# martius-lab/iCEM

Measured on AMD Instinct MI355X. Metric: traj-steps/sec (N x h), iCEM inner planning loop, higher is better.
Workload: dtype f32 storage; model step 2xfp16 planes (3 products), f32 accumulate

## Files before the change

### icem_amd/build.py

```python
import hashlib
import json
import os
import subprocess
import sys
from concurrent.futures import ThreadPoolExecutor

HERE = os.path.dirname(os.path.abspath(__file__))
CSRC = os.path.join(HERE, "csrc")
UNITS = ["generic_kernels.hip", "plan.hip", "abi.hip", "exchange.hip", "k_sample.hip", "k_rollout.hip", "k_merge.hip",
         "k_iter_small.hip", "icem_rssm.hip", "icem_rssm_split.hip", "k_rollout_wide.hip", "collective.hip", "k_rollout_ahead.hip",
         "k_rollout_wide_split.hip", "k_rollout_hn.hip"]
OUT = os.path.join(HERE, "libicem_hip.so")
OUT_FAULTS = os.path.join(HERE, "libicem_hip_faults.so")
FAULT_UNIT = "exchange.hip"
MARK = b"ICEM_BUILD_HASH="
OBJ = os.path.join(CSRC, "_obj")
FLAGS = ["--offload-arch=gfx950", "-O3", "-std=c++17", "-fPIC", "-Wno-unused-function"]
UNIT_FLAGS = {}
if os.environ.get("ICEM_DEV_SHAPES"):
    FLAGS.append(f"-DICEM_FAST_SHAPES(X)=X({os.environ['ICEM_DEV_SHAPES']})")


def _hipcc() -> str:
    return os.environ.get("HIPCC", "/opt/rocm/bin/hipcc")


def _units():
    return [u for u in UNITS if os.path.exists(os.path.join(CSRC, u))]


def _headers():
    hs = sorted(os.path.join(CSRC, f) for f in os.listdir(CSRC) if f.endswith(".h"))
    return hs + [os.path.join(os.path.dirname(HERE), "include", "icem_hip.h")]


def _digest(paths, extra=""):
    m = hashlib.sha256(extra.encode())
    for p in paths:
        m.update(os.path.basename(p).encode())
        with open(p, "rb") as f:
            m.update(f.read())
    return m.hexdigest()[:16]


def source_hash() -> str:
    return _digest([os.path.join(CSRC, u) for u in _units()] + _headers(), " ".join(FLAGS) + repr(sorted(UNIT_FLAGS.items())))


def embedded_hash(path: str = OUT):
    try:
        with open(path, "rb") as f:
            blob = f.read()
    except OSError:
        return None
    at = blob.find(MARK)
    if at < 0:
        return None
    tag = blob[at + len(MARK):at + len(MARK) + 16]
    return tag.decode() if len(tag) == 16 and all(c in b"0123456789abcdef" for c in tag) else None


def build_info() -> dict:
    info = {"source_hash": source_hash(), "built_from": embedded_hash(), "stale": True}
    info["stale"] = info["built_from"] != info["source_hash"]
    return info


def up_to_date() -> bool:
    return not build_info()["stale"]


def _object(unit, headers_digest, faults=False):
    src = os.path.join(CSRC, unit)
    extra = [f'-DICEM_BUILD_HASH="{source_hash()}"'] if unit == "abi.hip" else []
    if faults:
        extra.append("-DICEM_FAULT_INJECTION")
    cmd = [_hipcc(), *FLAGS, *UNIT_FLAGS.get(unit, []), *extra, "-I", CSRC, "-c", src]
    key = _digest([src], " ".join("csrc" if a == CSRC else a for a in cmd[1:-1]) + headers_digest)
    stem = os.path.splitext(unit)[0] + ("_faults" if faults else "")
    return cmd, os.path.join(OBJ, f"{stem}.{key}.o")


def object_path(unit: str) -> str:
    return _object(unit, _digest(_headers()))[1]


def _compile(unit, headers_digest, verbose, faults=False):
    cmd, obj = _object(unit, headers_digest, faults)
    stem = os.path.splitext(unit)[0] + ("_faults" if faults else "")
    if not os.path.exists(obj):
        for f in os.listdir(OBJ):
            if f.startswith(stem + ".") and f.endswith(".o"):
                os.remove(os.path.join(OBJ, f))
        if verbose:
            print(" ".join(cmd + ["-o", obj]), flush=True)
        subprocess.check_call(cmd + ["-o", obj + ".tmp"])
        os.replace(obj + ".tmp", obj)
    return obj


def build(force: bool = False, verbose: bool = True) -> str:
    if not force and up_to_date() and embedded_hash(OUT_FAULTS) == source_hash():
        return OUT
    os.makedirs(OBJ, exist_ok=True)
    if force:
        for f in os.listdir(OBJ):
            os.remove(os.path.join(OBJ, f))
    hd = _digest(_headers())
    with ThreadPoolExecutor(max_workers=min(8, os.cpu_count() or 1)) as ex:
        fut_faults = ex.submit(_compile, FAULT_UNIT, hd, verbose, True)
        objs = list(ex.map(lambda u: _compile(u, hd, verbose), _units()))
        obj_faults = fut_faults.result()
    objs_f = [obj_faults if os.path.basename(o).startswith(os.path.splitext(FAULT_UNIT)[0] + ".") else o for o in objs]
    for out, oo in ((OUT, objs), (OUT_FAULTS, objs_f)):
        cmd = [_hipcc(), "--offload-arch=gfx950", "-shared", "-fPIC", *oo, "-ldl", "-o", out]
        if verbose:
            print(" ".join(cmd), flush=True)
        subprocess.check_call(cmd)
    if embedded_hash() != source_hash():
        raise RuntimeError("libicem_hip.so does not carry the hash of the sources it was just built from")
    return OUT


if __name__ == "__main__":
    build(force="--force" in sys.argv)
    print(json.dumps(build_info()))
```

### icem_amd/csrc/k_iter_small.hip

```cpp
#include "fused_dev.h"

namespace icem {

namespace {

constexpr bool sr_quad(int d, int rw) { return rw <= 2 && ((4 * 16 * rw * d + 63) / 64) * 64 + 64 <= 1024; }
constexpr int sr_threads(int d, int rw) { return (((sr_quad(d, rw) ? 4 : 1) * 16 * rw * d + 63) / 64) * 64; }

template <int H, int D, int O, int KIND, int ROUNDS, int RW, int KREG, bool REC, int ARITH>
__device__ __forceinline__ void sample_rollout_body(const FastSampleArgs& sa, const FastRolloutArgs& ra, const MergeSingleArgs& am,
                                                    const PackPrev& ap) {
    constexpr bool PM = KREG > 0;
    constexpr bool QS = sr_quad(D, RW);
    constexpr bool T4 = QS && O <= 20 && sr_threads(D, RW) >= 256 * RW && ARITH == 0;
    using T16 = typename TileSel<H, D, O, KIND, ARITH>::type;
    using Tile = typename std::conditional<T4, Tile4<H, D, (O <= 20 ? O : 17), KIND>, T16>::type;
    constexpr int RWV = T4 ? 4 * RW : RW;
    constexpr int HD = H * D;
    constexpr int TPB = 16 * RW;
    constexpr int ROWS = TPB * D;
    constexpr int NT = sr_threads(D, RW);
    constexpr int NTT = NT + (PM ? 64 : 0);
    static_assert(NTT <= 1024 && HD % 2 == 0, "workgroup shape");
    constexpr int VW = HD % 4 == 0 ? 4 : 2;
    using Vec = typename VecOf<VW>::type;
    __shared__ __attribute__((aligned(16))) float ms[2 * HD];
    __shared__ __attribute__((aligned(16))) float tilebuf[T16::SLACK + TPB * HD + T16::TAIL];
    __shared__ unsigned long long wg_keys[2][RW][32];
    __shared__ float obs_stage[32];
    constexpr int WROWS = H / 2 + 1;
    __shared__ __attribute__((aligned(16))) float Wl[QS ? NT / 64 : 1][QS ? WROWS * WQ_STRIDE : 4];
    __shared__ unsigned long long sel[PM ? 64 : 1];
    __shared__ unsigned long long cand[PM ? 64 : 1];
    __shared__ int slot[PM ? 64 : 1];
    float* tile_rows = tilebuf + T16::SLACK;
    const int tid = threadIdx.x;
    const int lane = tid & 63;
    const int wave = tid >> 6;
    const int n_rows = ra.n_rows;
    const bool has_pack = PM && REC && ap.part_k != nullptr;
    if constexpr (PM && REC) {
        if (has_pack && blockIdx.x == 0) {
            MergeSingleArgs pk{};
            pk.n_lists = ap.n_lists;
            pk.n_pool = ap.n_pool;
            pk.n_global = ap.n_global;
            pk.K = ap.K;
            pk.h = H;
            pk.d = D;
            pk.part_k = ap.part_k;
            pk.actions = ap.actions;
            pk.n_keep = ap.n_keep;
            pk.elites_cost_cur = ap.keep_costs;
            pk.keep_base = ap.n_loc;
            __builtin_amdgcn_s_setprio(3);
            if (ra.dbg && tid == 0) ra.dbg[0] = wall_clock64();
            if (tid < 64) {
                if constexpr (NTT <= 512)
                    merge_select<12>(pk, lane, cand, sel);
                else
                    merge_select_stream(pk, lane, cand, sel);
            }
            __syncthreads();
            if (ra.dbg && tid == 0) ra.dbg[1] = wall_clock64();
            pack_records_body<12>(pk, ap.n_loc, ap.shard_lo, ap.records, ap.px, tilebuf, sel, tid, NTT);
            if (ra.dbg && tid == 0) ra.dbg[2] = wall_clock64();
            return;
        }
    }
    const int wg = blockIdx.x - (has_pack ? 1 : 0);
    const int n_wg = ra.list_wgs > 0 ? ra.list_wgs : (int)gridDim.x - (has_pack ? 1 : 0);
    const int base = wg * TPB;
    if (base >= n_rows) return;
    if (ra.dbg && tid == 0 && wg == 0) ra.dbg[8] = wall_clock64();
    const int rowi = QS ? tid >> 2 : tid, q = tid & 3;
    const int nl = rowi / D, jd = rowi - nl * D;
    const bool has_row = rowi < ROWS;
    float* trow = tile_rows + nl * HD + jd;
    const float* mrow = ms + jd;
    Tile tile;
    float obs_reg = 0.f;
    constexpr int WPL = (WROWS * HMAX + 63) / 64;
    float wreg[QS ? WPL : 1];
    const bool pre_drawn = !PM && sa.raw_src != nullptr;
    if constexpr (QS) {
        if (tid < NT && !pre_drawn) {
#pragma unroll
            for (int i = 0; i < WPL; ++i) wreg[i] = sa.W[(i * 64 + lane) < WROWS * HMAX ? i * 64 + lane : 0];
        }
    }
    const int r_mine = base + nl;
    float lo_reg = 0.f, hi_reg = 0.f;
    if ((PM || pre_drawn) && tid < NT) {
        lo_reg = sa.low[jd];
        hi_reg = sa.high[jd];
    }
    constexpr int NVR = !PM ? (TPB * (HD / VW) + NTT - 1) / NTT : 1;
    constexpr int NVB = NVR < 4 ? NVR : 4;
    constexpr int NEL = !PM && QS ? (H - 1 + 3) / 4 : 1;
    typedef float RawV __attribute__((ext_vector_type(VW)));
    RawV rawv[NVB];
    float elv[NEL];
    if (!PM) {
        const int total4 = (n_rows - base < TPB ? n_rows - base : TPB) * (HD / VW);
        RawV* t4 = reinterpret_cast<RawV*>(tile_rows);
        float mreg[(HD + NTT - 1) / NTT], sreg[(HD + NTT - 1) / NTT];
#pragma unroll
        for (int i = 0; i < (HD + NTT - 1) / NTT; ++i) {
            const int e = tid + i * NTT;
            mreg[i] = sa.mean[e < HD ? e : 0];
            sreg[i] = sa.std[e < HD ? e : 0];
        }
        if (pre_drawn) {
            const RawV* g4 = reinterpret_cast<const RawV*>(sa.raw_src + (size_t)base * HD);
#pragma unroll
            for (int i = 0; i < NVB; ++i) {
                const int e = tid + i * NTT;
                rawv[i] = g4[e < total4 ? e : 0];
            }
            if constexpr (QS) {
                if (has_row && tid < NT && r_mine >= sa.n && r_mine < n_rows) {
                    const float* src = sa.elites_src + (size_t)(r_mine - sa.n) * HD + jd;
#pragma unroll
                    for (int i = 0; i < NEL; ++i) elv[i] = src[(q + 4 * i < H - 1 ? q + 4 * i + 1 : 1) * D];
                }
            }
        }
        obs_reg = ra.obs0[(tid < 32 && tid < ra.o) ? tid : 0];
        if (wave < RWV) tile.load(ra, lane);
#pragma unroll
        for (int i = 0; i < (HD + NTT - 1) / NTT; ++i) {
            const int e = tid + i * NTT;
            if (e < HD) {
                ms[e] = mreg[i];
                ms[HD + e] = sreg[i];
            }
        }
        if (pre_drawn) {
#pragma unroll
            for (int i = 0; i < NVB; ++i) {
                const int e = tid + i * NTT;
                if (e < total4) t4[e] = rawv[i];
            }
            if constexpr (NVR > NVB) {
                const RawV* g4 = reinterpret_cast<const RawV*>(sa.raw_src + (size_t)base * HD);
                for (int e0 = tid + NVB * NTT; e0 < total4; e0 += NVB * NTT) {
#pragma unroll
                    for (int i = 0; i < NVB; ++i) rawv[i] = g4[e0 + i * NTT < total4 ? e0 + i * NTT : 0];
#pragma unroll
                    for (int i = 0; i < NVB; ++i)
                        if (e0 + i * NTT < total4) t4[e0 + i * NTT] = rawv[i];
                }
            }
        }
        __syncthreads();
    }
    if (ra.dbg && tid == 0 && wg == 0) ra.dbg[9] = wall_clock64();
    if (pre_drawn) {
        if (has_row && tid < NT) {
            const float lo = lo_reg, hi = hi_reg;
            constexpr int QN = QS ? 4 : 1;
            const int q0 = QS ? q : 0;
            if (r_mine < sa.n) {
                for (int t = q0; t < H; t += QN) {
                    const float v = __builtin_fmaf(trow[t * D], mrow[HD + t * D], mrow[t * D]);
                    trow[t * D] = __builtin_amdgcn_fmed3f(v, lo, hi);
                }
            } else if (r_mine < n_rows) {
                const float* src = sa.elites_src + (size_t)(r_mine - sa.n) * HD + jd;
                if ((H - 1) % QN == q0) {
                    const float v = __builtin_fmaf(trow[(H - 1) * D], mrow[HD + (H - 1) * D], mrow[(H - 1) * D]);
                    trow[(H - 1) * D] = __builtin_amdgcn_fmed3f(v, lo, hi);
                }
                if constexpr (QS) {
#pragma unroll
                    for (int i = 0; i < NEL; ++i)
                        if (q + 4 * i < H - 1) trow[(q + 4 * i) * D] = elv[i];
                } else {
                    for (int t = q0; t < H - 1; t += QN) trow[t * D] = src[(t + 1) * D];
                }
            } else {
                for (int t = q0; t < H; t += QN) trow[t * D] = 0.f;
            }
        }
    } else
    if constexpr (QS) {
        if (tid < NT) {
            float* wl = Wl[wave];
            sample_into_tile_quad<H, D, ROUNDS, PM>(sa, has_row, n_rows, r_mine, jd, q, trow, mrow, wl, [&]() {
#pragma unroll
                for (int i = 0; i < WPL; ++i) {
                    const int e = i * 64 + lane;
                    if (e < WROWS * HMAX) wl[(e / HMAX) * WQ_STRIDE + (e % HMAX)] = wreg[i];
                }
                __builtin_amdgcn_fence(__ATOMIC_RELEASE, "wavefront");
                __builtin_amdgcn_wave_barrier();
                __builtin_amdgcn_fence(__ATOMIC_ACQUIRE, "wavefront");
            });
        }
    } else if (has_row) {
        sample_into_tile<H, D, ROUNDS, PM>(sa, n_rows, r_mine, jd, trow, mrow);
    }
    if constexpr (PM) {
        if (tid >= NT) {
            if constexpr (RW <= 4) __builtin_amdgcn_s_setprio(3);
            if constexpr (REC) {
                if (ra.dbg && lane == 0 && wg == 0) ra.dbg[3] = wall_clock64();
            }
            else if constexpr (RW >= 8)
                merge_select_stream(am, lane, cand, sel);
            else
                merge_select_shallow<3>(am, lane, cand, sel);
        }
    }
    if (PM) {
        obs_reg = ra.obs0[(tid < 32 && tid < ra.o) ? tid : 0];
        if (wave < RWV) tile.load(ra, lane);
    }
    const float* rd0 = nullptr;
    if constexpr (!T4) rd0 = tile.read_ptr(tilebuf + (wave < RW ? wave : 0) * 16 * HD, lane, HD);
    if constexpr (PM) {
        const MergeSingleArgs& m = am;
        if constexpr (REC) {
            merge_select_records_wg(am, tid >= NT, lane, tid, NTT, sel, slot, (ra.dbg && wg == 0) ? ra.dbg + 7 : nullptr);
            if (ra.dbg && tid == 0 && wg == 0) ra.dbg[4] = wall_clock64();
        } else {
            __syncthreads();
        }
        if (ra.dbg && tid == 0 && wg == 0) ra.dbg[5] = wall_clock64();
        if (!REC && ra.dbg && tid == 0 && wg == 0) ra.dbg[15] = wall_clock64();
        const float* rows[KREG > 0 ? KREG : 1];
        merge_rows<KREG, REC>(m, sel, slot, rows);
        for (int e = tid; e < HD; e += NTT) {
            float xs[KREG > 0 ? KREG : 1];
#pragma unroll
            for (int r = 0; r < KREG; ++r) xs[r] = rows[r][e];
            float nm, ns;
            refit_element_regs<float, KREG>(m.K, m.alpha, m.mean[e], m.std[e], xs, nm, ns);
            ms[e] = nm;
            ms[HD + e] = ns;
            if (wg == 0) {
                m.mean_out[e] = nm;
                m.std_out[e] = ns;
#pragma unroll
                for (int r = 0; r < KREG; ++r)
                    if (r < m.K) m.elites_next[(size_t)r * HD + e] = xs[r];
            }
        }
        if (wg == 0 && tid < m.K) m.elites_cost_next[tid] = key_cost(sel[tid]);
        __syncthreads();
        if (ra.dbg && tid == 0 && wg == 0) ra.dbg[6] = wall_clock64();
        if (!REC && ra.dbg && tid == 0 && wg == 0) ra.dbg[7] = wall_clock64();
        if (has_row && r_mine < sa.n) {
            const float lo = lo_reg, hi = hi_reg;
            for (int t = QS ? q : 0; t < H; t += QS ? 4 : 1) {
                const float v = __builtin_fmaf(trow[t * D], mrow[HD + t * D], mrow[t * D]);
                trow[t * D] = __builtin_amdgcn_fmed3f(v, lo, hi);
            }
        }
    }
    if (tid < 32) {
        float ov = obs_reg;
        asm volatile("" : "+v"(ov));
        obs_stage[tid] = tid < ra.o ? ov : 0.f;
    }
    if (ra.dbg && tid == 0 && wg == 0) ra.dbg[10] = wall_clock64();
    __syncthreads();
    if (sa.row0_mean && sa.first_index + base == 0) {
        for (int e = tid; e < HD; e += NTT) tile_rows[e] = ms[e];
        __syncthreads();
    }
    {
        const int total4 = (n_rows - base < TPB ? n_rows - base : TPB) * (HD / VW);
        const Vec* t4 = reinterpret_cast<const Vec*>(tile_rows);
        Vec* g4 = reinterpret_cast<Vec*>(sa.out + (size_t)base * HD);
        constexpr int CP0 = (NTT - 64 * RWV >= 128) ? 64 * RWV : 0;
        if (tid >= CP0)
            for (int e = tid - CP0; e < total4; e += NTT - CP0) g4[e] = t4[e];
    }
    if (ra.dbg && tid == 0 && wg == 0) ra.dbg[11] = wall_clock64();
    unsigned long long run_key = KEY_SENTINEL;
    if constexpr (T4) {
        if (wave < RWV) {
            tile.load_obs(obs_stage);
            const int rs = wave * 4 + (lane >> 4);
            const int row = base + rs;
            const float* rd = tile.read_ptr(tilebuf, rs, HD);
            const float* ar = tile.row_ptr(tilebuf, rs, HD);
            typename Tile::State st;
            tile.init(st);
#pragma unroll
            for (int t = 0; t < H; ++t) tile.step(st, rd + t * D, ar + t * D);
            const float cost = tile.cost(st);
            const bool live = row < n_rows;
            if ((lane & 15) == 0) {
                if (live) ra.costs[row] = cost;
                note_nonfinite(ra, cost, live);
                wg_keys[0][0][rs] = (live && row < ra.n_cand) ? make_key(cost, row)
                                    : TPB <= 16 ? KEY_SENTINEL : ((KEY_SENTINEL & 0xFFFFFFFF00000000ull) | (KEY_FILL_LO + (unsigned)rs));
            }
        }
        if (ra.dbg && tid == 0 && wg == 0) ra.dbg[13] = wall_clock64();
        if (ra.K > 0 && wg < n_wg) {
            __syncthreads();
            if (wave == 0 && TPB <= 16) {
                const unsigned long long key = wave_sort_first<16>(lane < TPB ? wg_keys[0][0][lane] : KEY_SENTINEL, lane);
                if (lane < ra.K) {
                    if (ra.part_k) {
                        ra.part_k[(size_t)lane * n_wg + wg] = key;
                    } else {
                        ra.part_c[(size_t)wg * ra.K + lane] = key_cost(key);
                        ra.part_i[(size_t)wg * ra.K + lane] = key_idx(key);
                    }
                }
            } else if (wave == 0) {
                constexpr int NK = TPB <= 16 ? 16 : 32, PARTS = 64 / NK, PER = NK / PARTS;
                static_assert(TPB <= 32 && PER % 2 == 0, "one wave counts for the slab");
                const unsigned long long* keys = &wg_keys[0][0][0];
                const int i = lane & (NK - 1), part = lane / NK;
                const unsigned long long mine = i < TPB ? keys[i] : KEY_SENTINEL;
                unsigned place = 0;
#pragma unroll
                for (int c = 0; c < PER; ++c) {
                    const int e = part * PER + c;
                    place += (e < TPB && keys[e < TPB ? e : 0] < mine) ? 1u : 0u;
                }
                if (NK == 16) place += (unsigned)__shfl_xor((int)place, 16, 64);
                place += (unsigned)__shfl_xor((int)place, 32, 64);
                if (part == 0 && i < TPB && place < (unsigned)ra.K) {
                    const bool filler = (mine >> 32) == (KEY_SENTINEL >> 32) && (unsigned)mine >= KEY_FILL_LO;
                    const unsigned long long key = filler ? KEY_SENTINEL : mine;
                    if (ra.part_k) {
                        ra.part_k[(size_t)place * n_wg + wg] = key;
                    } else {
                        ra.part_c[(size_t)wg * ra.K + place] = key_cost(key);
                        ra.part_i[(size_t)wg * ra.K + place] = key_idx(key);
                    }
                }
            }
        }
    } else {
        if (wave < RW) {
            tile.load_obs(obs_stage);
            run_key = rollout_slab<Tile, H, D, true>(tile, ra, rd0, base + wave * 16 + (lane & 15), n_rows, run_key, true, lane);
            if (ra.dbg && tid == 0 && wg == 0) ra.dbg[12] = wall_clock64();
        }
        if (ra.dbg && tid == 0 && wg == 0) ra.dbg[13] = wall_clock64();
        if (ra.K > 0 && wg < n_wg) wg_merge_emit<RW>(wg_keys, run_key, ra.K, lane, wave, ra, wg, n_wg);
    }
    if (ra.dbg && tid == 0 && wg == 0) ra.dbg[14] = wall_clock64();
}


template <int H, int D, int O, int KIND, int ROUNDS, int RW, int KREG, bool REC, int ARITH>
__global__ __launch_bounds__(sr_threads(D, RW) + (KREG > 0 ? 64 : 0)) void sample_rollout_kernel(FastIterArgs a) {
    sample_rollout_body<H, D, O, KIND, ROUNDS, RW, KREG, REC, ARITH>(a.s, a.r, a.m, a.p);
}

template <int H, int D, int O, int KIND, int ROUNDS, int RW, int KREG, int ARITH>
__global__ __launch_bounds__(sr_threads(D, RW) + (KREG > 0 ? 64 : 0)) void sample_rollout_batch_kernel(const FastIterArgs* __restrict__ args,
                                                                                                      BatchBases bases) {
    const FastIterArgs& a = args[blockIdx.y];
    FastSampleArgs s = from_device(a.s);
    const unsigned long long base = bases.v[blockIdx.y];
    add_base64(s.off_lo, s.off_hi, base);
    add_base64(s.off2_lo, s.off2_hi, base);
    const FastRolloutArgs r = from_device(a.r);
    const MergeSingleArgs m = from_device(a.m);
    sample_rollout_body<H, D, O, KIND, ROUNDS, RW, KREG, false, ARITH>(s, r, m, a.p);
}

}

constexpr int single_launch_max_rw(int h, int d) {
    int best = 0;
    for (int rw = 1; rw <= 8; rw *= 2)
        if (sr_threads(d, rw) + 64 <= 1024 && 16 * rw * h * d * 4 <= 120 * 1024) best = rw;
    return best;
}

static bool sample_rollout_shape(int h, int d, int O, int rounds, int n_rows, int n_tail, int* grid_out, int* rw_out,
                                 int* tail_out = nullptr) {
    const int max_rw = opt_i(OPT_FUSE_MAX_RW);
    int grid, rw, tail = 0;
    r16_shape(n_rows, &grid, &rw);
    const int mult = g_batch.mult;
    if (mult > 1) {
        int g_all, rw_all;
        r16_shape(n_rows * mult, &g_all, &rw_all);
        const int cap = opt_i(OPT_BATCH_MAX_RW);
        rw = std::min(std::max(rw, rw_all), std::min(cap > 0 ? cap : 8, single_launch_max_rw(h, d)));
        while (rw > 1 && rw > single_launch_max_rw(h, d)) rw /= 2;
        grid = (std::max(1, (n_rows + 15) / 16) + rw - 1) / rw;
        if (grid > FAST_MAX_LISTS) return false;
    } else
    if (n_tail > 0 && n_tail <= 64) {
        int g2, w2;
        r16_shape(n_rows - n_tail, &g2, &w2);
        if (w2 < rw && sr_threads(d, w2) + 64 <= 512 && g2 == FAST_MAX_LISTS && n_rows - n_tail == FAST_MAX_LISTS * 16 * w2) {
            rw = w2;
            tail = n_tail;
        }
    }
    if (rounds != 10 || rw > max_rw || n_rows <= 0 || !fast_rollout_supported(h, d, O, 1) || !fast_sample_supported(h, d))
        return false;
    if (rw > single_launch_max_rw(h, d)) return false;
    *grid_out = tail ? (n_rows + 16 * rw - 1) / (16 * rw) : std::min(grid, (n_rows + 16 * rw - 1) / (16 * rw));
    *rw_out = rw;
    if (tail_out) *tail_out = tail;
    return true;
}

int sample_rollout_lists(int h, int d, int O, int rounds, int n_rows, int n_tail, int* tail_out) {
    int grid, rw, tail = 0;
    if (!sample_rollout_shape(h, d, O, rounds, n_rows, n_tail, &grid, &rw, &tail)) return 0;
    if (tail_out) *tail_out = tail;
    return tail ? FAST_MAX_LISTS : grid;
}

bool sample_rollout_merge_ok(int h, int d, int O, int rounds, int n_rows, int K) {
    const int on = opt_i(OPT_MERGE_PROLOGUE);
    int grid, rw;
    return on && K + 1 <= 12 && sample_rollout_shape(h, d, O, rounds, n_rows, 0, &grid, &rw);
}

bool sample_rollout_pack_ok(int h, int d, int O, int rounds, int n_rows, int K) {
    const int on = opt_i(OPT_RIDING_PACK);
    int grid, rw;
    return on && sample_rollout_merge_ok(h, d, O, rounds, n_rows, K) && sample_rollout_shape(h, d, O, rounds, n_rows, 0, &grid, &rw) &&
           K * (h * d + 2) <= 16 * rw * h * d;
}

void launch_sample_rollout(const FastIterArgs& a, int h, int d, int O, int kind, bool merge_prologue, hipStream_t st) {
    int grid, rw;
    if (!sample_rollout_shape(h, d, O, 10, a.r.n_rows, a.r.list_wgs > 0 ? a.s.n_shift : 0, &grid, &rw)) return;
    if (g_batch.rec) {
        if (merge_prologue && a.m.records) {
            g_batch.unsupported = true;
            return;
        }
        BatchRecord r;
        r.kind = BATCH_SAMPLE_ROLLOUT;
        r.it = a;
        r.h = h, r.d = d, r.O = O, r.model_kind = kind, r.rw = rw, r.grid = grid;
        r.prologue = merge_prologue;
        g_batch.rec->push_back(r);
        return;
    }
    if (merge_prologue && a.m.records && a.p.part_k) grid += 1;
#define XK(HH, DD, OO, WW, KR, RC)                                                                                      \
    {                                                                                                                   \
        constexpr int NT = sr_threads(DD, WW) + (KR > 0 ? 64 : 0);                                                     \
        if constexpr (OO <= 20) {                                                                                       \
            if (a.r.arith == 1) {                                                                                       \
                if (kind == 1)                                                                                          \
                    hipLaunchKernelGGL((sample_rollout_kernel<HH, DD, OO, 1, 10, WW, KR, RC, 1>), dim3(grid), dim3(NT), 0, st, a); \
                else                                                                                                    \
                    hipLaunchKernelGGL((sample_rollout_kernel<HH, DD, OO, 0, 10, WW, KR, RC, 1>), dim3(grid), dim3(NT), 0, st, a); \
                return;                                                                                                 \
            }                                                                                                           \
        }                                                                                                               \
        if (kind == 1)                                                                                                  \
            hipLaunchKernelGGL((sample_rollout_kernel<HH, DD, OO, 1, 10, WW, KR, RC, 0>), dim3(grid), dim3(NT), 0, st, a); \
        else                                                                                                            \
            hipLaunchKernelGGL((sample_rollout_kernel<HH, DD, OO, 0, 10, WW, KR, RC, 0>), dim3(grid), dim3(NT), 0, st, a); \
        return;                                                                                                         \
    }
#define XW(HH, DD, OO, WW)                                                   \
    if constexpr (WW <= single_launch_max_rw(HH, DD)) {                      \
        if (rw == WW) {                                                      \
            if (merge_prologue && a.m.records) XK(HH, DD, OO, WW, 12, true)  \
            if (merge_prologue) XK(HH, DD, OO, WW, 12, false)                \
            XK(HH, DD, OO, WW, 0, false)                                     \
        }                                                                    \
    }
#define XR(HH, DD, OO)                   \
    if (h == HH && d == DD && O == OO) { \
        XW(HH, DD, OO, 1)                \
        XW(HH, DD, OO, 2)                \
        XW(HH, DD, OO, 4)                \
        XW(HH, DD, OO, 8)                \
    }
    ICEM_FAST_SHAPES(XR)
#undef XR
#undef XW
#undef XK
}

void launch_sample_rollout_batch(const BatchRecord& s, const FastIterArgs* args_dev, const BatchBases& bases, int n, hipStream_t st) {
    const int h = s.h, d = s.d, O = s.O, kind = s.model_kind, rw = s.rw, arith = s.it.r.arith;
    const dim3 grid(s.grid, n);
#define XK(HH, DD, OO, WW, KR)                                                                                          \
    {                                                                                                                   \
        constexpr int NT = sr_threads(DD, WW) + (KR > 0 ? 64 : 0);                                                     \
        if constexpr (OO <= 20) {                                                                                       \
            if (arith == 1) {                                                                                           \
                if (kind == 1)                                                                                          \
                    hipLaunchKernelGGL((sample_rollout_batch_kernel<HH, DD, OO, 1, 10, WW, KR, 1>), grid, dim3(NT), 0, st, args_dev, bases); \
                else                                                                                                    \
                    hipLaunchKernelGGL((sample_rollout_batch_kernel<HH, DD, OO, 0, 10, WW, KR, 1>), grid, dim3(NT), 0, st, args_dev, bases); \
                return;                                                                                                 \
            }                                                                                                           \
        }                                                                                                               \
        if (kind == 1)                                                                                                  \
            hipLaunchKernelGGL((sample_rollout_batch_kernel<HH, DD, OO, 1, 10, WW, KR, 0>), grid, dim3(NT), 0, st, args_dev, bases); \
        else                                                                                                            \
            hipLaunchKernelGGL((sample_rollout_batch_kernel<HH, DD, OO, 0, 10, WW, KR, 0>), grid, dim3(NT), 0, st, args_dev, bases); \
        return;                                                                                                         \
    }
#define XW(HH, DD, OO, WW)                                  \
    if constexpr (WW <= single_launch_max_rw(HH, DD)) {     \
        if (rw == WW) {                                     \
            if (s.prologue) XK(HH, DD, OO, WW, 12)          \
            XK(HH, DD, OO, WW, 0)                           \
        }                                                   \
    }
#define XR(HH, DD, OO)                   \
    if (h == HH && d == DD && O == OO) { \
        XW(HH, DD, OO, 1)                \
        XW(HH, DD, OO, 2)                \
        XW(HH, DD, OO, 4)                \
        XW(HH, DD, OO, 8)                \
    }
    ICEM_FAST_SHAPES(XR)
#undef XR
#undef XW
#undef XK
}

}
```

### icem_amd/csrc/k_merge.hip

```cpp
#include "fused_dev.h"
#include "refit.h"

namespace icem {

namespace {

template <int KREG, bool REC>
__device__ __forceinline__ void merge_single_body(const MergeSingleArgs& a, unsigned char* smem_raw) {
    __shared__ unsigned long long sel[64];
    __shared__ unsigned long long cand[64];
    __shared__ int slot[64];
    typedef float __attribute__((address_space(3))) * LdsF;
    const LdsF new_mean = (LdsF)smem_raw;
    const int tid = threadIdx.x;
    const int lane = tid & 63;
    const int hd = a.h * a.d;
    if (a.dbg && threadIdx.x == 0) a.dbg[0] = wall_clock64();
    constexpr int EPL = 4;
    const bool pre = hd <= MERGE_WG * EPL;
    float om[EPL], os[EPL], blo[EPL], bhi[EPL];
#pragma unroll
    for (int i = 0; i < EPL; ++i) {
        const int e = tid + i * MERGE_WG;
        om[i] = (pre && e < hd) ? a.mean[e] : 0.f;
        os[i] = (pre && e < hd) ? a.std[e] : 0.f;
    }
    auto request_bounds = [&]() {
#pragma unroll
        for (int i = 0; i < EPL; ++i) {
            const int e = tid + i * MERGE_WG;
            blo[i] = (pre && a.last && e < hd) ? a.low[e % a.d] : 0.f;
            bhi[i] = (pre && a.last && e < hd) ? a.high[e % a.d] : 0.f;
        }
    };
    if (REC || tid >= 64) request_bounds();
    if constexpr (REC) {
        merge_select_records_wg(a, tid < 64, lane, tid, MERGE_WG, sel, slot);
        if (a.dbg && threadIdx.x == 0) a.dbg[4] = wall_clock64();
    } else {
        if (tid < 64) merge_select_shallow<3>(a, lane, cand, sel);
        if (a.dbg && threadIdx.x == 0) a.dbg[4] = wall_clock64();
        if (tid < 64) request_bounds();
        __syncthreads();
    }
    const float* rows[KREG];
    merge_rows<KREG, REC>(a, sel, slot, rows);
    float best0 = 0.f;
    auto finish_one = [&](int e, float old_mean, float old_std) {
        float xs[KREG];
#pragma unroll
        for (int r = 0; r < KREG; ++r) xs[r] = rows[r][e];
#pragma unroll
        for (int r = 0; r < KREG; ++r) asm volatile("" : "+v"(xs[r]));
        float nm, ns;
        refit_element_regs<float, KREG>(a.K, a.alpha, old_mean, old_std, xs, nm, ns);
#pragma unroll
        for (int r = 0; r < KREG; ++r)
            if (r < a.K) a.elites_next[(size_t)r * hd + e] = xs[r];
        if (!a.last) {
            a.mean_out[e] = nm;
            a.std_out[e] = ns;
        } else {
            new_mean[e] = nm;
        }
        if (e == tid) best0 = xs[0];
    };
    if (pre) {
#pragma unroll
        for (int i = 0; i < EPL; ++i) {
            const int e = tid + i * MERGE_WG;
            if (e < hd) finish_one(e, om[i], os[i]);
        }
    } else {
        for (int e = tid; e < hd; e += MERGE_WG) finish_one(e, a.mean[e], a.std[e]);
    }
    if (a.dbg && threadIdx.x == 0) a.dbg[5] = wall_clock64();
    if (tid < a.K) a.elites_cost_next[tid] = key_cost(sel[tid]);
    if (a.last) {
        __syncthreads();
        if (pre) {
#pragma unroll
            for (int i = 0; i < EPL; ++i) {
                const int e = tid + i * MERGE_WG;
                if (e < hd) {
                    a.mean_out[e] = (e + a.d < hd) ? new_mean[e + a.d] : new_mean[e];
                    a.std_out[e] = (bhi[i] - blo[i]) / 2.f * a.init_std;
                }
            }
        } else {
            for (int e = tid; e < hd; e += MERGE_WG) {
                const int j = e % a.d;
                a.mean_out[e] = (e + a.d < hd) ? new_mean[e + a.d] : new_mean[e];
                a.std_out[e] = (a.high[j] - a.low[j]) / 2.f * a.init_std;
            }
        }
        if (tid < a.d) a.executed[tid] = best0;
        if (tid == 0) a.best_cost[0] = key_cost(sel[0]);
    }
    if (a.dbg && threadIdx.x == 0) a.dbg[6] = wall_clock64();
}

template <int KREG, bool REC>
__global__ __launch_bounds__(MERGE_WG) void merge_single_kernel(MergeSingleArgs a) {
    extern __shared__ __attribute__((aligned(16))) unsigned char smem_raw[];
    merge_single_body<KREG, REC>(a, smem_raw);
}

template <int H, int KREG>
__global__ __launch_bounds__(MERGE_WG) void merge_noise_kernel(MergeSingleArgs a, FastSampleArgs z1, FastSampleArgs z2, int wgs1) {
    extern __shared__ __attribute__((aligned(16))) unsigned char smem_raw[];
    if (blockIdx.x == 0) {
        merge_single_body<KREG, false>(a, smem_raw);
        return;
    }
    const bool second = (int)blockIdx.x > wgs1;
    const FastSampleArgs& z = second ? z2 : z1;
    float* tile = reinterpret_cast<float*>(smem_raw);
    const int d = z.d, hd = H * d, tpw = MERGE_WG / d, tid = threadIdx.x;
    const int n_base = ((int)blockIdx.x - 1 - (second ? wgs1 : 0)) * tpw;
    const int n_here = cmin(tpw, z.n - n_base);
    if (tid < n_here * d) {
        const int nl = tid / d;
        const int j = tid - nl * d;
        float* trow = tile + nl * hd + j;
        sample_row<H, 10>(z.W, (unsigned)(z.first_index + n_base + nl), (unsigned)j, z.off_lo, z.off_hi, z.seed_lo, z.seed_hi,
                          [&](int t, float y) { trow[t * d] = y; }, z.white != 0);
    }
    __syncthreads();
    float* gdst = z.out + (size_t)n_base * hd;
    const int total = n_here * hd;
    if ((hd & 3) == 0) {
        const float4* t4 = reinterpret_cast<const float4*>(tile);
        float4* g4 = reinterpret_cast<float4*>(gdst);
        for (int e = tid; e < total / 4; e += MERGE_WG) g4[e] = t4[e];
    } else {
        for (int e = tid; e < total; e += MERGE_WG) gdst[e] = tile[e];
    }
}

template <int H, int KREG>
__global__ __launch_bounds__(MERGE_WG) void merge_noise_batch_kernel(const MergeNoiseBatchArgs* __restrict__ args, BatchBases bases, int wgs1) {
    extern __shared__ __attribute__((aligned(16))) unsigned char smem_raw[];
    const MergeNoiseBatchArgs& g = args[blockIdx.y];
    if (blockIdx.x == 0) {
        const MergeSingleArgs a = from_device(g.a);
        merge_single_body<KREG, false>(a, smem_raw);
        return;
    }
    const bool second = (int)blockIdx.x > wgs1;
    const FastSampleArgs z = from_device(second ? g.z2 : g.z1);
    float* tile = reinterpret_cast<float*>(smem_raw);
    const int d = z.d, hd = H * d, tpw = MERGE_WG / d, tid = threadIdx.x;
    const int n_base = ((int)blockIdx.x - 1 - (second ? wgs1 : 0)) * tpw;
    const int n_here = cmin(tpw, z.n - n_base);
    if (n_here <= 0) return;
    uint32_t off_lo = z.off_lo, off_hi = z.off_hi;
    add_base64(off_lo, off_hi, bases.v[blockIdx.y]);
    if (tid < n_here * d) {
        const int nl = tid / d;
        const int j = tid - nl * d;
        float* trow = tile + nl * hd + j;
        sample_row<H, 10>(z.W, (unsigned)(z.first_index + n_base + nl), (unsigned)j, off_lo, off_hi, z.seed_lo, z.seed_hi,
                          [&](int t, float y) { trow[t * d] = y; }, z.white != 0);
    }
    __syncthreads();
    float* gdst = z.out + (size_t)n_base * hd;
    const int total = n_here * hd;
    if ((hd & 3) == 0) {
        const float4* t4 = reinterpret_cast<const float4*>(tile);
        float4* g4 = reinterpret_cast<float4*>(gdst);
        for (int e = tid; e < total / 4; e += MERGE_WG) g4[e] = t4[e];
    } else {
        for (int e = tid; e < total; e += MERGE_WG) gdst[e] = tile[e];
    }
}

constexpr size_t PACK_STAGE_MAX = 48 * 1024;

template <int KREG>
__global__ __launch_bounds__(MERGE_WG) void pack_records_kernel(MergeSingleArgs a, int n_loc, int shard_lo, float* records, XchgPush px) {
    __shared__ unsigned long long sel[64];
    __shared__ unsigned long long cand[64];
    extern __shared__ __attribute__((aligned(16))) float stage[];
    const int tid = threadIdx.x;
    if (tid < 64) merge_select<KREG>(a, tid, cand, sel);
    __syncthreads();
    pack_records_body<KREG>(a, n_loc, shard_lo, records, px, stage, sel, tid, MERGE_WG);
}

template <int KREG>
__global__ __launch_bounds__(MERGE_WG) void pack_merge_kernel(MergeSingleArgs pk, int n_loc, int shard_lo, float* records, XchgPush px,
                                                               MergeSingleArgs m) {
    __shared__ unsigned long long sel[64];
    __shared__ unsigned long long cand[64];
    extern __shared__ __attribute__((aligned(16))) unsigned char smem_raw[];
    const int tid = threadIdx.x;
    if (tid < 64) merge_select<KREG>(pk, tid, cand, sel);
    __syncthreads();
    pack_records_body<KREG>(pk, n_loc, shard_lo, records, px, reinterpret_cast<float*>(smem_raw), sel, tid, MERGE_WG);
    __syncthreads();
    merge_single_body<KREG, true>(m, smem_raw);
}

__global__ __launch_bounds__(1024) void topk_small_kernel(const float* costs, int n, int K, float* out_c, int* out_i) {
    __shared__ unsigned long long wg_keys[2][16][32];
    const int lane = threadIdx.x & 63, wave = threadIdx.x >> 6;
    unsigned long long run = KEY_SENTINEL;
    bool first = true;
    for (int base = wave * 64; base < n; base += 1024) {
        const int i = base + lane;
        unsigned long long key = wave_sort64(i < n ? make_key(costs[i], i) : KEY_SENTINEL, lane);
        if (!first) {
            const unsigned long long prev = __shfl(run, lane - 32, 64);
            key = (lane >= 32 && lane < 32 + K) ? prev : (lane < K ? key : KEY_SENTINEL);
            key = wave_sort64(key, lane);
        }
        run = key;
        first = false;
    }
    FastRolloutArgs fr{};
    fr.part_c = out_c;
    fr.part_i = out_i;
    wg_merge_emit<16>(wg_keys, run, K, lane, wave, fr, 0, 1);
}

__global__ __launch_bounds__(1024) void update_small_kernel(UpdateSmallArgs a) {
    __shared__ unsigned long long wg_keys[2][16][32];
    __shared__ unsigned long long sel[32];
    const int tid = threadIdx.x, lane = tid & 63, wave = tid >> 6;
    const int n_all = a.n + a.n_keep;
    unsigned long long run = KEY_SENTINEL;
    bool first = true;
    for (int base = wave * 64; base < n_all; base += 1024) {
        const int i = base + lane;
        unsigned long long key = KEY_SENTINEL;
        if (i < n_all) key = make_key(i < a.n ? a.costs[i] : a.keep_costs[i - a.n], i);
        key = wave_sort64(key, lane);
        if (!first) {
            const unsigned long long prev = __shfl(run, lane - 32, 64);
            key = (lane >= 32 && lane < 32 + a.K) ? prev : (lane < a.K ? key : KEY_SENTINEL);
            key = wave_sort64(key, lane);
        }
        run = key;
        first = false;
    }
    FastRolloutArgs fr{};
    fr.part_k = sel;
    wg_merge_emit<16>(wg_keys, run, a.K, lane, wave, fr, 0, 1);
    __syncthreads();
    if (tid < a.K) {
        a.elite_costs_out[tid] = key_cost(sel[tid]);
        a.idx_out[tid] = key_idx(sel[tid]);
    }
    auto row = [&](int r) -> const float* {
        int i = key_idx(sel[r]);
        if (i < 0 || i == INT_MAX) i = key_idx(sel[0]);
        return i < a.n ? a.pool + (size_t)i * a.hd : a.keep_actions + (size_t)(i - a.n) * a.hd;
    };
    for (int e = tid; e < a.hd; e += 1024) {
        for (int r = 0; r < a.K; ++r) a.elites_out[(size_t)r * a.hd + e] = row(r)[e];
        float nm, ns;
        refit_element<float>(a.K, a.alpha, a.mean[e], a.std[e], [&](int r) { return row(r)[e]; }, nm, ns);
        a.mean[e] = nm;
        a.std[e] = ns;
    }
}

}

void launch_update_small(const UpdateSmallArgs& a, hipStream_t st) {
    hipLaunchKernelGGL(update_small_kernel, dim3(1), dim3(1024), 0, st, a);
}

bool topk_small_ok(int n, int K) { return n >= 1 && n <= 16384 && K >= 1 && K <= 32; }

void launch_topk_small(const float* costs, int n, int K, float* out_c, int* out_i, hipStream_t st) {
    hipLaunchKernelGGL(topk_small_kernel, dim3(1), dim3(1024), 0, st, costs, n, K, out_c, out_i);
}

bool pack_can_push(int K, int h, int d) { return (size_t)K * (h * d + 2) * sizeof(float) <= PACK_STAGE_MAX; }

void launch_pack_records(const MergeSingleArgs& a, int n_loc, int shard_lo, float* records, hipStream_t st, const XchgPush& px) {
    const size_t lds = px.peers ? (size_t)a.K * (a.h * a.d + 2) * sizeof(float) : 0;
    if (a.K + 1 <= 12)
        hipLaunchKernelGGL((pack_records_kernel<12>), dim3(1), dim3(MERGE_WG), lds, st, a, n_loc, shard_lo, records, px);
    else
        hipLaunchKernelGGL((pack_records_kernel<34>), dim3(1), dim3(MERGE_WG), lds, st, a, n_loc, shard_lo, records, px);
}

void launch_pack_merge(const MergeSingleArgs& pk, int n_loc, int shard_lo, float* records, const XchgPush& px, const MergeSingleArgs& m,
                       hipStream_t st) {
    const size_t lds = std::max(px.peers ? (size_t)pk.K * (pk.h * pk.d + 2) : (size_t)0, (size_t)m.h * m.d) * sizeof(float);
    if (pk.K + 1 <= 12)
        hipLaunchKernelGGL((pack_merge_kernel<12>), dim3(1), dim3(MERGE_WG), lds, st, pk, n_loc, shard_lo, records, px, m);
    else
        hipLaunchKernelGGL((pack_merge_kernel<34>), dim3(1), dim3(MERGE_WG), lds, st, pk, n_loc, shard_lo, records, px, m);
}

bool merge_noise_ok(const MergeSingleArgs& a, int rounds) {
    return a.records == nullptr && a.K + 1 <= 12 && rounds == 10 && fast_sample_supported(a.h, a.d);
}

void launch_merge_noise(const MergeSingleArgs& a, const FastSampleArgs& z, const FastSampleArgs& z2, hipStream_t st) {
    if (g_batch.rec) {
        BatchRecord r;
        r.kind = BATCH_MERGE_NOISE;
        r.m = a;
        r.z1 = z;
        r.z2 = z2;
        g_batch.rec->push_back(r);
        return;
    }
    const int tpw = MERGE_WG / z.d;
    const int wgs1 = (z.n + tpw - 1) / tpw, wgs2 = z2.n > 0 ? (z2.n + tpw - 1) / tpw : 0;
    const int grid = 1 + wgs1 + wgs2;
    const size_t lds = std::max((size_t)a.h * a.d, (size_t)tpw * z.h * z.d) * sizeof(float);
#define X(HH)                                                                                                    \
    if (a.h == HH) {                                                                                             \
        hipLaunchKernelGGL((merge_noise_kernel<HH, 12>), dim3(grid), dim3(MERGE_WG), lds, st, a, z, z2, wgs1);   \
        return;                                                                                                  \
    }
    ICEM_FAST_HORIZONS(X)
#undef X
}

void launch_merge_batch(const BatchRecord& s, const MergeNoiseBatchArgs* args_dev, const BatchBases& bases, int n, hipStream_t st) {
    const MergeSingleArgs& a = s.m;
    int wgs1 = 0, wgs2 = 0, tpw = 1;
    if (s.kind == BATCH_MERGE_NOISE) {
        tpw = MERGE_WG / s.z1.d;
        wgs1 = (s.z1.n + tpw - 1) / tpw;
        wgs2 = s.z2.n > 0 ? (s.z2.n + tpw - 1) / tpw : 0;
    }
    const dim3 grid(1 + wgs1 + wgs2, n);
    const size_t lds = std::max((size_t)a.h * a.d, s.kind == BATCH_MERGE_NOISE ? (size_t)tpw * s.z1.h * s.z1.d : (size_t)0) * sizeof(float);
#define X(HH)                                                                                                              \
    if (a.h == HH) {                                                                                                       \
        hipLaunchKernelGGL((merge_noise_batch_kernel<HH, 12>), grid, dim3(MERGE_WG), lds, st, args_dev, bases, wgs1);      \
        return;                                                                                                            \
    }
    ICEM_FAST_HORIZONS(X)
#undef X
}

void launch_merge_single(const MergeSingleArgs& a, hipStream_t st) {
    if (g_batch.rec) {
        if (a.records || a.K + 1 > 12) {
            g_batch.unsupported = true;
            return;
        }
        BatchRecord r;
        r.kind = BATCH_MERGE_SINGLE;
        r.m = a;
        g_batch.rec->push_back(r);
        return;
    }
    const size_t lds = (size_t)a.h * a.d * sizeof(float);
    if (a.records) {
        if (a.K + 1 <= 12)
            hipLaunchKernelGGL((merge_single_kernel<12, true>), dim3(1), dim3(MERGE_WG), lds, st, a);
        else
            hipLaunchKernelGGL((merge_single_kernel<34, true>), dim3(1), dim3(MERGE_WG), lds, st, a);
    } else if (a.K + 1 <= 12) {
        hipLaunchKernelGGL((merge_single_kernel<12, false>), dim3(1), dim3(MERGE_WG), lds, st, a);
    } else {
        hipLaunchKernelGGL((merge_single_kernel<34, false>), dim3(1), dim3(MERGE_WG), lds, st, a);
    }
}

}
```

Baseline: 7.635 billion.

## Preload hot kernel arguments into SGPRs and defer cold argument block loads

Enables LLVM kernarg preloading on the iteration and merge kernels and reshapes their signatures so the most-used fields (pointers, seeds, packed counts) come first as scalar parameters. The large argument struct follows them and is read lazily through the kernarg segment pointer, after the sampling and merge-select prologue. The goal is to cut the kernel-entry latency of scalar loads from the argument segment in these short, latency-bound kernels. The cost is fragile offset arithmetic, bit-packed counts with range checks that skip the launch on overflow, and debug timestamp instrumentation that was reshuffled.

```diff
diff --git a/icem_amd/build.py b/icem_amd/build.py
--- a/icem_amd/build.py
+++ b/icem_amd/build.py
@@ -16,7 +16,8 @@
 MARK = b"ICEM_BUILD_HASH="
 OBJ = os.path.join(CSRC, "_obj")
 FLAGS = ["--offload-arch=gfx950", "-O3", "-std=c++17", "-fPIC", "-Wno-unused-function"]
-UNIT_FLAGS = {}
+_PRELOAD = ["-mllvm", "-amdgpu-kernarg-preload-count=16"]
+UNIT_FLAGS = {"k_iter_small.hip": _PRELOAD, "k_merge.hip": _PRELOAD}
 if os.environ.get("ICEM_DEV_SHAPES"):
     FLAGS.append(f"-DICEM_FAST_SHAPES(X)=X({os.environ['ICEM_DEV_SHAPES']})")
 
diff --git a/icem_amd/csrc/k_iter_small.hip b/icem_amd/csrc/k_iter_small.hip
--- a/icem_amd/csrc/k_iter_small.hip
+++ b/icem_amd/csrc/k_iter_small.hip
@@ -1,4 +1,6 @@
 #include "fused_dev.h"
+
+#include <cstdio>
 
 namespace icem {
 
@@ -7,9 +9,9 @@
 constexpr bool sr_quad(int d, int rw) { return rw <= 2 && ((4 * 16 * rw * d + 63) / 64) * 64 + 64 <= 1024; }
 constexpr int sr_threads(int d, int rw) { return (((sr_quad(d, rw) ? 4 : 1) * 16 * rw * d + 63) / 64) * 64; }
 
-template <int H, int D, int O, int KIND, int ROUNDS, int RW, int KREG, bool REC, int ARITH>
+template <int H, int D, int O, int KIND, int ROUNDS, int RW, int KREG, bool REC, int ARITH, typename Late>
 __device__ __forceinline__ void sample_rollout_body(const FastSampleArgs& sa, const FastRolloutArgs& ra, const MergeSingleArgs& am,
-                                                    const PackPrev& ap) {
+                                                    const PackPrev& ap, Late&& late) {
     constexpr bool PM = KREG > 0;
     constexpr bool QS = sr_quad(D, RW);
     constexpr bool T4 = QS && O <= 20 && sr_threads(D, RW) >= 256 * RW && ARITH == 0;
@@ -30,6 +32,7 @@
     __shared__ float obs_stage[32];
     constexpr int WROWS = H / 2 + 1;
     __shared__ __attribute__((aligned(16))) float Wl[QS ? NT / 64 : 1][QS ? WROWS * WQ_STRIDE : 4];
+    __shared__ long long wave_done[PM ? NTT / 64 : 1];
     __shared__ unsigned long long sel[PM ? 64 : 1];
     __shared__ unsigned long long cand[PM ? 64 : 1];
     __shared__ int slot[PM ? 64 : 1];
@@ -38,6 +41,7 @@
     const int lane = tid & 63;
     const int wave = tid >> 6;
     const int n_rows = ra.n_rows;
+    const long long t_entry = wall_clock64();
     const bool has_pack = PM && REC && ap.part_k != nullptr;
     if constexpr (PM && REC) {
         if (has_pack && blockIdx.x == 0) {
@@ -69,10 +73,8 @@
         }
     }
     const int wg = blockIdx.x - (has_pack ? 1 : 0);
-    const int n_wg = ra.list_wgs > 0 ? ra.list_wgs : (int)gridDim.x - (has_pack ? 1 : 0);
     const int base = wg * TPB;
     if (base >= n_rows) return;
-    if (ra.dbg && tid == 0 && wg == 0) ra.dbg[8] = wall_clock64();
     const int rowi = QS ? tid >> 2 : tid, q = tid & 3;
     const int nl = rowi / D, jd = rowi - nl * D;
     const bool has_row = rowi < ROWS;
@@ -91,7 +93,7 @@
     }
     const int r_mine = base + nl;
     float lo_reg = 0.f, hi_reg = 0.f;
-    if ((PM || pre_drawn) && tid < NT) {
+    if (!PM && pre_drawn && tid < NT) {
         lo_reg = sa.low[jd];
         hi_reg = sa.high[jd];
     }
@@ -155,7 +157,10 @@
         }
         __syncthreads();
     }
-    if (ra.dbg && tid == 0 && wg == 0) ra.dbg[9] = wall_clock64();
+    if (!PM && ra.dbg && tid == 0 && wg == 0) {
+        ra.dbg[8] = t_entry;
+        ra.dbg[9] = wall_clock64();
+    }
     if (pre_drawn) {
         if (has_row && tid < NT) {
             const float lo = lo_reg, hi = hi_reg;
@@ -197,9 +202,14 @@
                 __builtin_amdgcn_wave_barrier();
                 __builtin_amdgcn_fence(__ATOMIC_ACQUIRE, "wavefront");
             });
+            if (PM && !REC && lane == 0) wave_done[wave] = wall_clock64();
         }
     } else if (has_row) {
         sample_into_tile<H, D, ROUNDS, PM>(sa, n_rows, r_mine, jd, trow, mrow);
+    }
+    if (PM && tid < NT) {
+        lo_reg = sa.low[jd];
+        hi_reg = sa.high[jd];
     }
     if constexpr (PM) {
         if (tid >= NT) {
@@ -211,8 +221,17 @@
                 merge_select_stream(am, lane, cand, sel);
             else
                 merge_select_shallow<3>(am, lane, cand, sel);
-        }
-    }
+            if (!REC && lane == 0) wave_done[wave] = wall_clock64();
+        }
+    }
+    {
+    FastSampleArgs late_s = sa;
+    FastRolloutArgs late_r = ra;
+    MergeSingleArgs late_m = am;
+    late(late_s, late_r, late_m);
+    const FastSampleArgs& sa = late_s;
+    const FastRolloutArgs& ra = late_r;
+    const MergeSingleArgs& am = late_m;
     if (PM) {
         obs_reg = ra.obs0[(tid < 32 && tid < ra.o) ? tid : 0];
         if (wave < RWV) tile.load(ra, lane);
@@ -227,7 +246,16 @@
         } else {
             __syncthreads();
         }
-        if (ra.dbg && tid == 0 && wg == 0) ra.dbg[5] = wall_clock64();
+        if (ra.dbg && tid == 0 && wg == 0) {
+            ra.dbg[8] = ra.dbg[9] = t_entry;
+            ra.dbg[5] = wall_clock64();
+            if constexpr (QS && !REC) {
+                long long last = 0;
+                for (int w = 0; w < NT / 64; ++w) last = wave_done[w] > last ? wave_done[w] : last;
+                ra.dbg[1] = last;
+                ra.dbg[2] = wave_done[NT / 64];
+            }
+        }
         if (!REC && ra.dbg && tid == 0 && wg == 0) ra.dbg[15] = wall_clock64();
         const float* rows[KREG > 0 ? KREG : 1];
         merge_rows<KREG, REC>(m, sel, slot, rows);
@@ -280,6 +308,7 @@
     }
     if (ra.dbg && tid == 0 && wg == 0) ra.dbg[11] = wall_clock64();
     unsigned long long run_key = KEY_SENTINEL;
+    const int n_wg = ra.list_wgs > 0 ? ra.list_wgs : (int)gridDim.x - (has_pack ? 1 : 0);
     if constexpr (T4) {
         if (wave < RWV) {
             tile.load_obs(obs_stage);
@@ -349,12 +378,98 @@
         if (ra.K > 0 && wg < n_wg) wg_merge_emit<RW>(wg_keys, run_key, ra.K, lane, wave, ra, wg, n_wg);
     }
     if (ra.dbg && tid == 0 && wg == 0) ra.dbg[14] = wall_clock64();
-}
-
-
+    }
+}
+
+
+constexpr uint32_t hot_counts(int K, int n_keep, int n_lists) {
+    return (uint32_t)K | ((uint32_t)n_keep << 8) | ((uint32_t)n_lists << 16);
+}
+constexpr uint32_t hot_rows(int n_rows, int n_sampled) { return (uint32_t)n_rows | ((uint32_t)(n_rows - n_sampled) << 24); }
+constexpr int HOT_BYTES = 14 * 4;
+static_assert(HOT_BYTES % alignof(FastIterArgs) == 0, "the block follows the preloaded dwords without padding");
+__device__ __forceinline__ const FastIterArgs* cold_args() {
+    typedef const __attribute__((address_space(4))) unsigned char* KernArg;
+    KernArg p = (KernArg)__builtin_amdgcn_kernarg_segment_ptr() + HOT_BYTES;
+    asm volatile("" : "+s"(p));
+    return (const FastIterArgs*)p;
+}
 template <int H, int D, int O, int KIND, int ROUNDS, int RW, int KREG, bool REC, int ARITH>
-__global__ __launch_bounds__(sr_threads(D, RW) + (KREG > 0 ? 64 : 0)) void sample_rollout_kernel(FastIterArgs a) {
-    sample_rollout_body<H, D, O, KIND, ROUNDS, RW, KREG, REC, ARITH>(a.s, a.r, a.m, a.p);
+__global__ __launch_bounds__(sr_threads(D, RW) + (KREG > 0 ? 64 : 0)) void sample_rollout_kernel(
+    const unsigned long long* part_k, const float* elites_cost_cur, const float* W, uint32_t seed_lo, uint32_t seed_hi, uint32_t off_lo,
+    uint32_t off_hi, uint32_t first_index_lo, uint32_t rows, int keep_index, uint32_t counts, FastIterArgs a) {
+    static_assert(KREG > 0, "the merge-prologue form");
+    static_assert(sizeof(part_k) + sizeof(elites_cost_cur) + sizeof(W) + sizeof(seed_lo) + sizeof(seed_hi) + sizeof(off_lo) +
+                          sizeof(off_hi) + sizeof(first_index_lo) + sizeof(rows) + sizeof(keep_index) + sizeof(counts) == HOT_BYTES,
+                  "cold_args() finds the block behind exactly these parameters");
+    const int n_rows = (int)(rows & 0xFFFFFF), n_sampled = n_rows - (int)(rows >> 24);
+    auto hot = [&](FastSampleArgs& s, FastRolloutArgs& r, MergeSingleArgs& m) __attribute__((always_inline)) {
+        s.W = W;
+        s.n = n_sampled;
+        s.first_index = (long long)(((unsigned long long)s.first_index & 0xFFFFFFFF00000000ull) | first_index_lo);
+        s.seed_lo = seed_lo, s.seed_hi = seed_hi, s.off_lo = off_lo, s.off_hi = off_hi;
+        r.n_rows = n_rows;
+        m.part_k = part_k;
+        m.elites_cost_cur = elites_cost_cur;
+        m.K = (int)(counts & 0xFF), m.n_keep = (int)((counts >> 8) & 0xFF), m.n_lists = (int)(counts >> 16);
+    };
+    FastSampleArgs s = a.s;
+    FastRolloutArgs r = a.r;
+    MergeSingleArgs m = a.m;
+    hot(s, r, m);
+    m.keep_base = m.n_global = keep_index;
+    sample_rollout_body<H, D, O, KIND, ROUNDS, RW, KREG, REC, ARITH>(
+        s, r, m, a.p, [&](FastSampleArgs& ls, FastRolloutArgs& lr, MergeSingleArgs& lm) __attribute__((always_inline)) {
+            const FastIterArgs* c = cold_args();
+            ls = c->s, lr = c->r, lm = c->m;
+            hot(ls, lr, lm);
+        });
+}
+
+template <int H, int D, int O, int KIND, int ROUNDS, int RW, int KREG, bool REC, int ARITH>
+__global__ __launch_bounds__(sr_threads(D, RW)) void sample_rollout_kernel(const float* mean, const float* std, const float* raw_src,
+                                                                           const float* obs0, const float* low, const float* high,
+                                                                           int n_rows, int n_sampled, FastIterArgs a) {
+    static_assert(KREG == 0, "the form without a merge prologue");
+    static_assert(sizeof(mean) + sizeof(std) + sizeof(raw_src) + sizeof(obs0) + sizeof(low) + sizeof(high) + sizeof(n_rows) +
+                          sizeof(n_sampled) == HOT_BYTES,
+                  "cold_args() finds the block behind exactly these parameters");
+    auto hot = [&](FastSampleArgs& s, FastRolloutArgs& r) __attribute__((always_inline)) {
+        s.mean = mean, s.std = std, s.raw_src = raw_src, s.low = low, s.high = high;
+        s.n = n_sampled;
+        r.obs0 = obs0;
+        r.n_rows = n_rows;
+    };
+    FastSampleArgs s = a.s;
+    FastRolloutArgs r = a.r;
+    hot(s, r);
+    sample_rollout_body<H, D, O, KIND, ROUNDS, RW, KREG, REC, ARITH>(
+        s, r, a.m, a.p, [&](FastSampleArgs& ls, FastRolloutArgs& lr, MergeSingleArgs& lm) __attribute__((always_inline)) {
+            const FastIterArgs* c = cold_args();
+            ls = c->s, lr = c->r, lm = c->m;
+            hot(ls, lr);
+        });
+}
+
+static_assert(FAST_MAX_LISTS <= 0xFFFF, "hot_counts: 16 bits of list count");
+template <int H, int D, int O, int KIND, int RW, int KREG, bool REC, int ARITH>
+static void launch_sr(int grid, const FastIterArgs& a, hipStream_t st) {
+    constexpr int NT = sr_threads(D, RW) + (KREG > 0 ? 64 : 0);
+    if constexpr (KREG > 0) {
+        const int n_shifted = a.r.n_rows - a.s.n, keep_index = a.m.keep_base >= 0 ? a.m.keep_base : a.m.n_global;
+        if (a.m.K < 0 || a.m.K > 0xFF || a.m.n_keep < 0 || a.m.n_keep > 0xFF || a.m.n_lists < 0 || a.m.n_lists > 0xFFFF ||
+            a.r.n_rows < 0 || a.r.n_rows > 0xFFFFFF || n_shifted < 0 || n_shifted > 0xFF || keep_index < 0) {
+            fprintf(stderr, "icem: sample_rollout_kernel not launched: K %d / n_keep %d / n_lists %d / rows %d (%d sampled) / kept index %d "
+                            "outside the packed arguments' range\n", a.m.K, a.m.n_keep, a.m.n_lists, a.r.n_rows, a.s.n, keep_index);
+            return;
+        }
+        hipLaunchKernelGGL((sample_rollout_kernel<H, D, O, KIND, 10, RW, KREG, REC, ARITH>), dim3(grid), dim3(NT), 0, st, a.m.part_k,
+                           a.m.elites_cost_cur, a.s.W, a.s.seed_lo, a.s.seed_hi, a.s.off_lo, a.s.off_hi, (uint32_t)a.s.first_index,
+                           hot_rows(a.r.n_rows, a.s.n), keep_index, hot_counts(a.m.K, a.m.n_keep, a.m.n_lists), a);
+    } else {
+        hipLaunchKernelGGL((sample_rollout_kernel<H, D, O, KIND, 10, RW, KREG, REC, ARITH>), dim3(grid), dim3(NT), 0, st, a.s.mean,
+                           a.s.std, a.s.raw_src, a.r.obs0, a.s.low, a.s.high, a.r.n_rows, a.s.n, a);
+    }
 }
 
 template <int H, int D, int O, int KIND, int ROUNDS, int RW, int KREG, int ARITH>
@@ -367,7 +482,8 @@
     add_base64(s.off2_lo, s.off2_hi, base);
     const FastRolloutArgs r = from_device(a.r);
     const MergeSingleArgs m = from_device(a.m);
-    sample_rollout_body<H, D, O, KIND, ROUNDS, RW, KREG, false, ARITH>(s, r, m, a.p);
+    sample_rollout_body<H, D, O, KIND, ROUNDS, RW, KREG, false, ARITH>(s, r, m, a.p,
+                                                                       [](FastSampleArgs&, FastRolloutArgs&, MergeSingleArgs&) {});
 }
 
 }
@@ -450,20 +566,19 @@
     if (merge_prologue && a.m.records && a.p.part_k) grid += 1;
 #define XK(HH, DD, OO, WW, KR, RC)                                                                                      \
     {                                                                                                                   \
-        constexpr int NT = sr_threads(DD, WW) + (KR > 0 ? 64 : 0);                                                     \
         if constexpr (OO <= 20) {                                                                                       \
             if (a.r.arith == 1) {                                                                                       \
                 if (kind == 1)                                                                                          \
-                    hipLaunchKernelGGL((sample_rollout_kernel<HH, DD, OO, 1, 10, WW, KR, RC, 1>), dim3(grid), dim3(NT), 0, st, a); \
+                    launch_sr<HH, DD, OO, 1, WW, KR, RC, 1>(grid, a, st);                                               \
                 else                                                                                                    \
-                    hipLaunchKernelGGL((sample_rollout_kernel<HH, DD, OO, 0, 10, WW, KR, RC, 1>), dim3(grid), dim3(NT), 0, st, a); \
+                    launch_sr<HH, DD, OO, 0, WW, KR, RC, 1>(grid, a, st);                                               \
                 return;                                                                                                 \
             }                                                                                                           \
         }                                                                                                               \
         if (kind == 1)                                                                                                  \
-            hipLaunchKernelGGL((sample_rollout_kernel<HH, DD, OO, 1, 10, WW, KR, RC, 0>), dim3(grid), dim3(NT), 0, st, a); \
+            launch_sr<HH, DD, OO, 1, WW, KR, RC, 0>(grid, a, st);                                                       \
         else                                                                                                            \
-            hipLaunchKernelGGL((sample_rollout_kernel<HH, DD, OO, 0, 10, WW, KR, RC, 0>), dim3(grid), dim3(NT), 0, st, a); \
+            launch_sr<HH, DD, OO, 0, WW, KR, RC, 0>(grid, a, st);                                                       \
         return;                                                                                                         \
     }
 #define XW(HH, DD, OO, WW)                                                   \
diff --git a/icem_amd/csrc/k_merge.hip b/icem_amd/csrc/k_merge.hip
--- a/icem_amd/csrc/k_merge.hip
+++ b/icem_amd/csrc/k_merge.hip
@@ -15,7 +15,7 @@
     const int tid = threadIdx.x;
     const int lane = tid & 63;
     const int hd = a.h * a.d;
-    if (a.dbg && threadIdx.x == 0) a.dbg[0] = wall_clock64();
+    const long long t_entry = wall_clock64();
     constexpr int EPL = 4;
     const bool pre = hd <= MERGE_WG * EPL;
     float om[EPL], os[EPL], blo[EPL], bhi[EPL];
@@ -36,10 +36,10 @@
     if (REC || tid >= 64) request_bounds();
     if constexpr (REC) {
         merge_select_records_wg(a, tid < 64, lane, tid, MERGE_WG, sel, slot);
-        if (a.dbg && threadIdx.x == 0) a.dbg[4] = wall_clock64();
+        if (a.dbg && threadIdx.x == 0) a.dbg[0] = t_entry, a.dbg[4] = wall_clock64();
     } else {
         if (tid < 64) merge_select_shallow<3>(a, lane, cand, sel);
-        if (a.dbg && threadIdx.x == 0) a.dbg[4] = wall_clock64();
+        if (a.dbg && threadIdx.x == 0) a.dbg[0] = t_entry, a.dbg[4] = wall_clock64();
         if (tid < 64) request_bounds();
         __syncthreads();
     }
@@ -100,17 +100,30 @@
     if (a.dbg && threadIdx.x == 0) a.dbg[6] = wall_clock64();
 }
 
+#define ICEM_MERGE_HOT_PARAMS                                                                                              \
+    const unsigned long long *hot_part_k, const float *hot_cost_cur, const float *hot_mean, const float *hot_std, int hot_n_lists, \
+        int hot_K, int hot_n_keep, int hot_h, int hot_d, int hot_last
+#define ICEM_MERGE_HOT_ARGS(a) (a).part_k, (a).elites_cost_cur, (a).mean, (a).std, (a).n_lists, (a).K, (a).n_keep, (a).h, (a).d, (a).last
+#define ICEM_MERGE_HOT_APPLY(m)                                                                                  \
+    (m).part_k = hot_part_k, (m).elites_cost_cur = hot_cost_cur, (m).mean = hot_mean, (m).std = hot_std, (m).n_lists = hot_n_lists, \
+    (m).K = hot_K, (m).n_keep = hot_n_keep, (m).h = hot_h, (m).d = hot_d, (m).last = hot_last
+
 template <int KREG, bool REC>
-__global__ __launch_bounds__(MERGE_WG) void merge_single_kernel(MergeSingleArgs a) {
+__global__ __launch_bounds__(MERGE_WG) void merge_single_kernel(ICEM_MERGE_HOT_PARAMS, MergeSingleArgs a) {
     extern __shared__ __attribute__((aligned(16))) unsigned char smem_raw[];
-    merge_single_body<KREG, REC>(a, smem_raw);
+    MergeSingleArgs m = a;
+    ICEM_MERGE_HOT_APPLY(m);
+    merge_single_body<KREG, REC>(m, smem_raw);
 }
 
 template <int H, int KREG>
-__global__ __launch_bounds__(MERGE_WG) void merge_noise_kernel(MergeSingleArgs a, FastSampleArgs z1, FastSampleArgs z2, int wgs1) {
+__global__ __launch_bounds__(MERGE_WG) void merge_noise_kernel(ICEM_MERGE_HOT_PARAMS, MergeSingleArgs a, FastSampleArgs z1, FastSampleArgs z2,
+                                                               int wgs1) {
     extern __shared__ __attribute__((aligned(16))) unsigned char smem_raw[];
     if (blockIdx.x == 0) {
-        merge_single_body<KREG, false>(a, smem_raw);
+        MergeSingleArgs m = a;
+        ICEM_MERGE_HOT_APPLY(m);
+        merge_single_body<KREG, false>(m, smem_raw);
         return;
     }
     const bool second = (int)blockIdx.x > wgs1;
@@ -317,7 +330,8 @@
     const size_t lds = std::max((size_t)a.h * a.d, (size_t)tpw * z.h * z.d) * sizeof(float);
 #define X(HH)                                                                                                    \
     if (a.h == HH) {                                                                                             \
-        hipLaunchKernelGGL((merge_noise_kernel<HH, 12>), dim3(grid), dim3(MERGE_WG), lds, st, a, z, z2, wgs1);   \
+        hipLaunchKernelGGL((merge_noise_kernel<HH, 12>), dim3(grid), dim3(MERGE_WG), lds, st, ICEM_MERGE_HOT_ARGS(a), a, z, \
+                           z2, wgs1);                                                                            \
         return;                                                                                                  \
     }
     ICEM_FAST_HORIZONS(X)
@@ -358,14 +372,14 @@
     const size_t lds = (size_t)a.h * a.d * sizeof(float);
     if (a.records) {
         if (a.K + 1 <= 12)
-            hipLaunchKernelGGL((merge_single_kernel<12, true>), dim3(1), dim3(MERGE_WG), lds, st, a);
+            hipLaunchKernelGGL((merge_single_kernel<12, true>), dim3(1), dim3(MERGE_WG), lds, st, ICEM_MERGE_HOT_ARGS(a), a);
         else
-            hipLaunchKernelGGL((merge_single_kernel<34, true>), dim3(1), dim3(MERGE_WG), lds, st, a);
+            hipLaunchKernelGGL((merge_single_kernel<34, true>), dim3(1), dim3(MERGE_WG), lds, st, ICEM_MERGE_HOT_ARGS(a), a);
     } else if (a.K + 1 <= 12) {
-        hipLaunchKernelGGL((merge_single_kernel<12, false>), dim3(1), dim3(MERGE_WG), lds, st, a);
-    } else {
-        hipLaunchKernelGGL((merge_single_kernel<34, false>), dim3(1), dim3(MERGE_WG), lds, st, a);
-    }
-}
-
-}
+        hipLaunchKernelGGL((merge_single_kernel<12, false>), dim3(1), dim3(MERGE_WG), lds, st, ICEM_MERGE_HOT_ARGS(a), a);
+    } else {
+        hipLaunchKernelGGL((merge_single_kernel<34, false>), dim3(1), dim3(MERGE_WG), lds, st, ICEM_MERGE_HOT_ARGS(a), a);
+    }
+}
+
+}
```

Result: faster. 7.961 billion, median of 6 (+4.3%).
